# apache/skywalking-banyandb

Measured on NVIDIA H100. Metric: measure datapoints scanned+aggregated/sec, higher is better.
Workload: dtype f64

## Files before the change

### skywalking-banyandb_b200/csrc/capi.cu

```cuda
#include <cuda_runtime.h>
#include <unistd.h>

#include <algorithm>
#include <atomic>
#include <cstdio>
#include <chrono>
#include <condition_variable>
#include <cstddef>
#include <cstdlib>
#include <deque>
#include <functional>
#include <thread>
#include <future>
#include <cstring>
#include <memory>
#include <type_traits>
#include <mutex>
#include <optional>
#include <string>
#include <unordered_map>
#include <vector>

#include "../../include/bydb_gpu.h"
#include "part_dir.hpp"
// ... 48 lines not shown
    uint8_t *d_unpack = nullptr;
    uint64_t unpacked_pages = 0, unpack_skipped = 0;
    uint8_t *d_dense = nullptr;
    uint64_t dense_pages = 0, dense_bytes = 0;
    const DevBlock *d_blocks = nullptr;
    const DevCol *d_cols = nullptr;
    const uint8_t *const *d_files = nullptr;
    uint64_t hbm_bytes = 0;
    int device = 0;
    cudaStream_t pool_stream = nullptr;
    ~Part() {
        if (pool_stream) {
            if (d_arena) cudaFreeAsync(d_arena, pool_stream);
            if (d_dir) cudaFreeAsync(d_dir, pool_stream);
            if (d_unpack) cudaFreeAsync(d_unpack, pool_stream);
            if (d_dense) cudaFreeAsync(d_dense, pool_stream);
        } else {
            if (d_arena) cudaFree(d_arena);
            if (d_dir) cudaFree(d_dir);
            if (d_unpack) cudaFree(d_unpack);
            if (d_dense) cudaFree(d_dense);
        }
    }
};

struct ZeroPage {
    uint32_t work_count, work_next;
    uint32_t err[2];
    unsigned long long stats[6];
    int32_t col_type[kMaxFcols];
    unsigned long long dd_counts[2];
    uint32_t slow_count, slow_next;
    uint32_t rest_count, rest_next;
};
static_assert(offsetof(ZeroPage, err) == 8 && offsetof(ZeroPage, stats) == 16 && offsetof(ZeroPage, col_type) == 64 &&
                  offsetof(ZeroPage, dd_counts) == 96 && offsetof(ZeroPage, slow_count) == 112 && offsetof(ZeroPage, rest_count) == 120,
              "zero page layout");
constexpr size_t kZeroPageBytes = 256;
static_assert(sizeof(ZeroPage) <= kZeroPageBytes, "zero page size");

struct ExecSlot {
    cudaStream_t stream = nullptr;
    static constexpr int kMaxBatches = 8;
    cudaEvent_t ev[4 * kMaxBatches] = {};
    uint8_t *pinned = nullptr;
    size_t pinned_bytes = 0;
    uint8_t *zpage = nullptr;
    ZeroPage *page(int batch) { return reinterpret_cast<ZeroPage *>(zpage + kZeroPageBytes * static_cast<size_t>(batch)); }
    bool express[kMaxBatches] = {};
    cudaEvent_t busy = nullptr;
    bool busy_pending = false;
    void wait_idle() {
        if (busy_pending) cudaEventSynchronize(busy);
        busy_pending = false;
    }
    static constexpr size_t kInitialPinned = 1u << 20;
    std::vector<uint8_t *> retired;
    int ensure_pinned(size_t n) {
        if (n <= pinned_bytes) return 0;
        size_t want = align_up(std::max(n, 2 * pinned_bytes), 1 << 16);
        uint8_t *fresh = nullptr;
        if (cudaMallocHost(reinterpret_cast<void **>(&fresh), want) != cudaSuccess) {
            cudaGetLastError();
            want = align_up(n, 1 << 16);
            if (cudaMallocHost(reinterpret_cast<void **>(&fresh), want) != cudaSuccess) return -1;
        }
        if (pinned) retired.push_back(pinned);
        pinned = fresh;
        pinned_bytes = want;
// ... 78 lines not shown
constexpr int kCommMaxRanks = 64;
constexpr size_t kCommCtl = 4096, kCommStatusOff = 1024, kCommDoneOff = 2048, kCommErrOff = 2056, kCommArgsOff = 2112;
struct Comm {
    int rank = -1, nranks = 0;
    uint8_t *mine = nullptr;
    size_t slot_bytes = 0, mailbox_bytes = 0;
    std::vector<uint8_t *> peer;
    std::vector<bool> ipc_opened;
    std::vector<size_t> peer_slot_bytes;
    uint64_t epoch = 0;
    std::vector<uint64_t> last_use;
    std::mutex mu;
    bool shared_device = false;
    cudaStream_t poll_stream = nullptr;
    unsigned long long *poll_buf = nullptr;
};

struct StageRing {
    static constexpr int kBufs = 3;
    static constexpr size_t kBytes = 64u << 20;
    uint8_t *buf[kBufs] = {};
    cudaEvent_t done[kBufs] = {};
    bool pending[kBufs] = {};
    int next = 0;
    std::mutex mu;
};

struct bydb_ctx {
    int device = 0;
    int sm_count = 0;
    int ctas_per_sm = 2;
    int ctas_per_sm_fast = 2;
    int ctas_per_sm_express = 2;
    uint64_t hbm_budget = 0;
    uint64_t hbm_used = 0;
    bool host_index = false;
    bool dense_pages = true;
    std::mutex mu;
    NameTable names;
    std::unordered_map<bydb_part_h, std::shared_ptr<Part>> parts;
    std::unordered_map<uint64_t, bydb_part_h> by_id;
    std::atomic<uint64_t> parts_gen{0};
    bydb_part_h next_handle = 1;
    std::vector<std::unique_ptr<ExecSlot>> free_slots;
    WorkPool pool;
    Comm comm;
    StageRing stage;
};

namespace {

int hbm_reserve(bydb_ctx *ctx, uint64_t bytes, const char *msg = "HBM budget exceeded") {
    std::lock_guard<std::mutex> lk(ctx->mu);
    if (ctx->hbm_budget && ctx->hbm_used + bytes > ctx->hbm_budget) return fail(BYDB_ENOMEM, msg);
    ctx->hbm_used += bytes;
    return 0;
}
void hbm_release(bydb_ctx *ctx, uint64_t bytes) {
    std::lock_guard<std::mutex> lk(ctx->mu);
    ctx->hbm_used -= bytes;
}

struct SlotLease {
    bydb_ctx *ctx;
    std::unique_ptr<ExecSlot> slot;
    SlotLease(bydb_ctx *c) : ctx(c) {
// ... 851 lines not shown
        sp.dd_index = reinterpret_cast<int32_t *>(d + off_dd_index);
        sp.dd_row_off = reinterpret_cast<unsigned long long *>(d + off_dd_rowoff);
        sp.dd_list = reinterpret_cast<uint32_t *>(d + off_dd_list);
        sp.dd_counts = z->dd_counts;
        CUDA_TRY(cudaMemsetAsync(sp.dd_index, 0xff, NB * 4, stream));
        launch_detect_overlap(sp, stream);
        CUDA_TRY(cudaMemcpyAsync(hz->dd_counts, z->dd_counts, sizeof hz->dd_counts, cudaMemcpyDeviceToHost, stream));
        CUDA_TRY(cudaStreamSynchronize(stream));
        const unsigned long long n_ddb = hz->dd_counts[0], n_ddr = hz->dd_counts[1];
        extra_launches += 1;
        if (stats) stats->d2h_bytes += sizeof hz->dd_counts;
        if (n_ddb > 0) {
            const size_t b_ts = align_up(n_ddr * 8, 256), b_sh = align_up(n_ddb * kMaskWords * 4, 256);
            CUDA_TRY(dd_scratch.alloc(2 * b_ts + b_sh, stream));
            sp.dd_ts = reinterpret_cast<int64_t *>(dd_scratch.base);
            sp.dd_ver = reinterpret_cast<int64_t *>(dd_scratch.base + b_ts);
            sp.dd_shadow = reinterpret_cast<uint32_t *>(dd_scratch.base + 2 * b_ts);
            sp.n_dd_blocks = static_cast<uint32_t>(n_ddb);
            launch_dedup(sp, ctx->sm_count * ctx->ctas_per_sm, stream);
            extra_launches += 2;
        }
        rp.dedup_done = 1;
    }
    {
        bool sums_only = q->n_preds == 0 && !overlap && NB > 0;
        for (size_t c = 0; c < F; ++c) sums_only = sums_only && (sp.fcol_need[c] & 2) == 0;
        slot.express[batch] = sums_only;
        if (sums_only) {
            sp.rest_list = reinterpret_cast<uint32_t *>(d + off_restlist);
            sp.rest_count = &z->rest_count;
            sp.rest_next = &z->rest_next;
            if (stats) stats->kernel_launches += 1;
        }
    }
    CUDA_TRY(cudaEventRecord(ev[1], stream));
    launch_scan_blocks(sp, ctx->sm_count * ctx->ctas_per_sm_express, ctx->sm_count * ctx->ctas_per_sm_fast, ctx->sm_count * ctx->ctas_per_sm, stream);
    CUDA_TRY(cudaEventRecord(ev[2], stream));
    launch_series_reduce(rp, stream);
    const int32_t *gstart = reinterpret_cast<const int32_t *>(h + st.off_gstart);
    bool small_groups = true;
    for (int32_t g = 0; g < G && small_groups; ++g) small_groups = gstart[g + 1] - gstart[g] <= 32;
    launch_group_reduce(rp, stream, small_groups);
    CUDA_TRY(cudaEventRecord(ev[3], stream));
    if (!resident) CUDA_TRY(cudaMemcpyAsync(hz, z, kZeroPageBytes, cudaMemcpyDeviceToHost, stream));
    if (stats) {
        stats->kernel_launches += (NB ? 1u : 0u) + 2u + (NS ? 1u : 0u) + 1u + extra_launches;
        if (!resident) stats->d2h_bytes += kZeroPageBytes;
    }
    return 0;
}

int read_zero_page(const ZeroPage &z, bool express, bydb_stats *stats) {
    if (stats) {
        stats->rows_scanned += z.stats[0];
        stats->rows_matched += z.stats[1];
        stats->page_bytes += z.stats[2];
        stats->blocks_scanned += z.stats[3];
        stats->blocks_slow_lane += static_cast<uint32_t>(z.stats[4]);
        stats->slow_lane_reasons |= static_cast<uint32_t>(z.stats[5]);
        stats->blocks_express_lane += express ? z.work_count - z.rest_count : 0u;
    }
    if (z.err[0] == 0) return 0;
    g_last_dev_err = z.err[0];
    char buf[96];
    snprintf(buf, sizeof buf, " (block/series #%u)", z.err[1]);
    return fail(dev_err_code(z.err[0]), std::string(dev_err_text(z.err[0])) + buf);
}

int collect_scan(ExecSlot &slot, bydb_stats *stats, int batch = 0) {
// ... 1642 lines not shown
    if (prop.major != 9 || prop.minor != 0)
        return fail(BYDB_ENOTSUP, std::string("device '") + prop.name + "' is not sm_90 (Hopper); this library is built for sm_90a only");
    auto ctx = new bydb_ctx();
    ctx->device = dev;
    ctx->sm_count = prop.multiProcessorCount;
    ctx->hbm_budget = cfg ? cfg->hbm_budget_bytes : 0;
    ctx->host_index = cfg && (cfg->flags & BYDB_CFG_HOST_INDEX) != 0;
    ctx->dense_pages = !(cfg && (cfg->flags & BYDB_CFG_NO_DENSE_PAGES) != 0);
    if (upload_pow10_table()) {
        delete ctx;
        return fail(BYDB_EIO, "cannot upload constant tables (is the library built for this GPU?)");
    }
    {
        cudaMemPool_t pool;
        if (cudaDeviceGetDefaultMemPool(&pool, dev) == cudaSuccess) {
            uint64_t thr = UINT64_MAX;
            cudaMemPoolSetAttribute(pool, cudaMemPoolAttrReleaseThreshold, &thr);
            int no = 0;
            cudaMemPoolSetAttribute(pool, cudaMemPoolReuseAllowInternalDependencies, &no);
        }
    }
    for (int i = 0; i < 2; ++i) {
        std::unique_ptr<ExecSlot> sl(new ExecSlot());
        if (sl->create() != 0) {
            cudaGetLastError();
            break;
        }
        ctx->free_slots.push_back(std::move(sl));
    }
    preload_kernels();
    preload_unpack_kernels();
    preload_index_kernels();
    preload_encode_kernels();
    int occ_express = 1, occ_fast = 1, occ_slow = 1;
    scan_max_ctas_per_sm(&occ_express, &occ_fast, &occ_slow);
    int want = (cfg && cfg->warps_per_sm > 0) ? (cfg->warps_per_sm + kWarpsPerCta - 1) / kWarpsPerCta : 64;
    ctx->ctas_per_sm = std::max(1, std::min(want, occ_slow));
    ctx->ctas_per_sm_fast = std::max(1, std::min(want, occ_fast));
    ctx->ctas_per_sm_express = std::max(1, std::min(want, occ_express));
    *out = ctx;
    return 0;
    });
}

void bydb_shutdown(bydb_ctx *ctx) {
    if (!ctx) return;
    cudaSetDevice(ctx->device);
    cudaDeviceSynchronize();
    ctx->free_slots.clear();
    ctx->parts.clear();
    for (int i = 0; i < StageRing::kBufs; ++i) {
        if (ctx->stage.buf[i]) cudaFreeHost(ctx->stage.buf[i]);
        if (ctx->stage.done[i]) cudaEventDestroy(ctx->stage.done[i]);
    }
    for (size_t r = 0; r < ctx->comm.peer.size(); ++r)
        if (ctx->comm.ipc_opened[r] && ctx->comm.peer[r]) cudaIpcCloseMemHandle(ctx->comm.peer[r]);
    if (ctx->comm.mine) cudaFree(ctx->comm.mine);
    if (ctx->comm.poll_stream) cudaStreamDestroy(ctx->comm.poll_stream);
    if (ctx->comm.poll_buf) cudaFreeHost(ctx->comm.poll_buf);
    delete ctx;
}

int bydb_part_register(bydb_ctx *ctx, uint64_t part_id, const bydb_part_files *files, bydb_part_h *out) {
    return guarded([&]() -> int {
    if (!ctx || !out) return fail(BYDB_EINVAL, "ctx/out is NULL");
    {
        std::lock_guard<std::mutex> lk(ctx->mu);
        auto it = ctx->by_id.find(part_id);
        if (it != ctx->by_id.end()) {
            *out = it->second;
            return 0;
        }
// ... 1718 lines not shown
```

### skywalking-banyandb_b200/csrc/scan_kernels.cu

```cuda
#include "scan_kernels.cuh"
#include "lane_decode.cuh"

#include <atomic>
#include <cfloat>
#include <cmath>
#include <cstring>

#include "../../include/bydb_gpu.h"

namespace bydb {

__constant__ double c_pow10[309];

__device__ __forceinline__ uint32_t smem_u32(const void *p) { return static_cast<uint32_t>(__cvta_generic_to_shared(p)); }

__device__ __forceinline__ void mbar_init(uint64_t *bar, uint32_t count) {
    asm volatile("mbarrier.init.shared::cta.b64 [%0], %1;" ::"r"(smem_u32(bar)), "r"(count) : "memory");
}
__device__ __forceinline__ void mbar_expect_tx(uint64_t *bar, uint32_t bytes) {
    asm volatile("mbarrier.arrive.expect_tx.shared::cta.b64 _, [%0], %1;" ::"r"(smem_u32(bar)), "r"(bytes) : "memory");
}
__device__ __forceinline__ bool mbar_try_wait(uint64_t *bar, uint32_t parity) {
    uint32_t ok;
    asm volatile(
// ... 1963 lines not shown
    swar_begin(sl, pw);
#pragma unroll
    for (int q = 0; q < 2; ++q) {
        const uint4 wa = *reinterpret_cast<const uint4 *>(src + 32 * q), wb = *reinterpret_cast<const uint4 *>(src + 32 * q + 16);
        swar_step<kClasses, false>(sl, wa.x, 0u);
        swar_step<kClasses, false>(sl, wa.y, 0u);
        swar_step<kClasses, false>(sl, wa.z, 0u);
        swar_step<kClasses, false>(sl, wa.w, 0u);
        swar_step<kClasses, false>(sl, wb.x, 0u);
        swar_step<kClasses, false>(sl, wb.y, 0u);
        swar_step<kClasses, false>(sl, wb.z, 0u);
        swar_step<kClasses, false>(sl, wb.w, 0u);
    }
}
struct ExpressUnit {
    int32_t Ta, Ra, Tb, Rb;
    uint32_t n;
    bool wide;
};
template <int kClasses>
__device__ __forceinline__ ExpressUnit express_unit(const uint8_t *src, uint32_t pwa, uint32_t pwb) {
    ExpressUnit r;
    SwarLane sl;
    express_half<kClasses>(sl, src, pwa);
    uint32_t wide = sl.wide;
    const uint32_t na = swar_end(sl, r.Ta, r.Ra);
    express_half<kClasses>(sl, src + kSwarChunkBytes, pwb);
    wide |= sl.wide;
    r.n = na | (swar_end(sl, r.Tb, r.Rb) << 16);
    r.wide = __any_sync(0xffffffffu, (wide & 0x80808080u) != 0);
    return r;
}

__global__ void __launch_bounds__(kWarpsPerCta * 32, BYDB_EXPRESS_CTAS) scan_sum_express_kernel(const __grid_constant__ ScanParams p) {
    extern __shared__ __align__(128) uint8_t smem_raw[];
    const int lane = threadIdx.x & 31;
    const int warp = threadIdx.x >> 5;
    ExpressSmem *sm = reinterpret_cast<ExpressSmem *>(smem_raw) + warp;
    if (lane == 0) {
        sm->fault = 0;
        for (int s = 0; s < kExpressStages; ++s) mbar_init(&sm->bar[s], 1);
        asm volatile("fence.mbarrier_init.release.cluster;" ::: "memory");
    }
    __syncthreads();
    const uint32_t nwork = *p.work_count;
    uint32_t seq = 0;
    unsigned long long st_rows = 0, st_bytes = 0;
    uint32_t st_blocks = 0, known_types = 0;
    for (;;) {
        uint32_t nb = 0;
        const uint32_t base = grab_work(p.work_next, nwork, kExpressBatch, nb, lane);
        if (nb == 0) break;
        const bool mine = static_cast<uint32_t>(lane) < nb;
        uint32_t g = 0, count = 0, col_begin = 0, n_cols = 0, pi = 0;
        bool ok = mine;
        if (mine) {
            g = p.worklist[base + lane];
            while (pi + 1 < p.n_parts && g >= p.parts[pi + 1].block_base) ++pi;
            const DevBlock *b = p.parts[pi].blocks + (g - p.parts[pi].block_base);
            count = b->count;
            col_begin = b->col_begin;
            n_cols = b->n_cols;
            ok = p.tmin <= b->ts_min && p.tmax >= b->ts_max && count >= 1;
        }
        uint32_t page_bytes = 0;
        for (uint32_t c = 0; c < p.n_fcols; ++c) {
            const uint8_t *abase = nullptr;
            uint32_t pstart = 0, pend = 0, total = 0, nst = 0, dense_b = 0;
            int64_t first = 0;
            int exp = 0;
            bool has_page = false, is_float = false, count_only = false, dense = false;
            if (ok) {
                const DevCol *cols = p.parts[pi].cols + col_begin;
                DevCol col{};
                bool found = false;
                uint32_t ci = 0;
                for (uint32_t i = 0; i < n_cols && !found; ++i) {
                    const DevCol cc = cols[i];
                    if (cc.name_id == p.fcol_name[c]) {
                        col = cc;
                        found = true;
                        ci = i;
                    }
                }
                if (found) {
                    is_float = col.value_type == BYDB_VT_FLOAT64;
                    if (!is_float && col.value_type != BYDB_VT_INT64) {
                        ok = false;
                    } else if (!check_col_type(p, c, col.value_type, known_types)) {
                        ok = false;
                    }
                    const uint8_t *page = p.parts[pi].files[col.file_id] + col.off;
                    const uint32_t hdr = is_float ? 11u : 9u;
                    if (ok && p.fcol_need[c] == 0) {
                        if (col.size < 2 || __ldg(page) == 9 || (__ldg(page) == kEncRawCells && __ldg(page + 1))) ok = false;
                        count_only = ok;
                        page_bytes += 1;
                    } else if (ok && p.parts[pi].dense && p.parts[pi].dense[col_begin + ci].n == count) {
                        const DevDense dd = p.parts[pi].dense[col_begin + ci];
                        exp = dd.exp;
                        first = dd.min;
                        dense_b = dd.b;
                        abase = dd.planes;
                        pend = total = dd.plane_bytes;
                        nst = (total + kExpressStageBytes - 1) / kExpressStageBytes;
                        has_page = true;
                        dense = true;
                        page_bytes += col.size;
                    } else if (ok) {
                        if (col.size < hdr || __ldg(page) != 3) {
                            ok = false;
                        } else {
                            if (is_float) exp = static_cast<int16_t>((static_cast<uint32_t>(__ldg(page + 1)) << 8) | __ldg(page + 2));
                            first = conv_bytes_to_int64(page + hdr - 8);
                            const uintptr_t a = reinterpret_cast<uintptr_t>(page + hdr);
                            abase = reinterpret_cast<const uint8_t *>(a & ~static_cast<uintptr_t>(15));
                            pstart = static_cast<uint32_t>(a & 15);
                            pend = pstart + (col.size - hdr);
                            total = (pend + 15u) & ~15u;
                            nst = pend > pstart ? (total + kExpressStageBytes - 1) / kExpressStageBytes : 0;
                            has_page = true;
                            page_bytes += col.size;
                        }
                    }
                }
            }
            const bool streams = ok && has_page && nst > 0;
            uint32_t sb = streams ? nst : 0;
#pragma unroll
            for (int sft = 1; sft < static_cast<int>(kExpressBatch); sft <<= 1) {
                const uint32_t o = __shfl_up_sync(0xffffffffu, sb, sft);
                if (lane >= sft) sb += o;
            }
            const uint32_t ts = __shfl_sync(0xffffffffu, sb, kExpressBatch - 1);
            sb -= streams ? nst : 0;
            const uint32_t seq0 = seq;
            auto issue = [&](uint32_t s) {
                const uint32_t bal = __ballot_sync(0xffffffffu, streams && s >= sb && s < sb + nst);
                const int src = __ffs(bal) - 1;
                const uint64_t ab = shfl_u64(reinterpret_cast<uint64_t>(abase), src);
                const uint32_t tot = __shfl_sync(0xffffffffu, total, src);
                const uint32_t off = (s - __shfl_sync(0xffffffffu, sb, src)) * kExpressStageBytes;
                if (lane == 0) ring_fill(sm, seq0 + s, reinterpret_cast<const uint8_t *>(ab) + off, min(static_cast<uint32_t>(kExpressStageBytes), tot - off));
            };
            __syncwarp();
            for (uint32_t s = 0; s < ts && s < static_cast<uint32_t>(kExpressStages); ++s) issue(s);
            seq += ts;
            for (uint32_t k = 0; k < nb; ++k) {
                const bool okk = __shfl_sync(0xffffffffu, ok, k);
                if (!okk) continue;
                const bool pagek = __shfl_sync(0xffffffffu, has_page, k);
                const bool cok = __shfl_sync(0xffffffffu, count_only, k);
                const uint32_t count_k = __shfl_sync(0xffffffffu, count, k);
                AggAcc acc;
                acc.init();
                bool good = true;
                if (pagek) {
                    const uint32_t nst_k = __shfl_sync(0xffffffffu, nst, k), sb_k = __shfl_sync(0xffffffffu, sb, k);
                    const uint32_t ps_k = __shfl_sync(0xffffffffu, pstart, k), pe_k = __shfl_sync(0xffffffffu, pend, k);
// ... 54 lines not shown
#endif
                        }
                        if (!dense_k && j == nst_k - 1 && lane == 0) last_byte = buf[(pe_k - 1) % kExpressStageBytes];
                        __syncwarp();
                        const uint32_t nx = s + kExpressStages;
                        if (nx < ts) {
                            if (j + kExpressStages < nst_k) {
                                const uint32_t off = (j + kExpressStages) * kExpressStageBytes;
                                if (lane == 0) ring_fill(sm, seq0 + nx, ab_k + off, min(static_cast<uint32_t>(kExpressStageBytes), tot_k - off));
                            } else {
                                issue(nx);
                            }
                        }
                    }
                    last_byte = __shfl_sync(0xffffffffu, last_byte, 0);
                    const int32_t zeros_after = static_cast<int32_t>(nst_k * kExpressStageBytes - pe_k);
                    if (dense_k) good = true;
                    else if (nst_k == 0) good = count_k == 1;
                    else good = good && tb - zeros_after + 1 == static_cast<int32_t>(count_k) && last_byte < 0x80u;
#if !BYDB_EXPRESS_DECODE
                    good = true;
#endif
                    uint64_t us = U + static_cast<uint64_t>(S);
#pragma unroll
                    for (int m = 16; m >= 1; m >>= 1) us += shfl_xor_u64(us, m);
                    acc.add_scaled(first_k, count_k);
                    acc.lo += us;
                    acc.hi += (dense_k ? 0 : (static_cast<int64_t>(us) >> 63)) + (acc.lo < us ? 1 : 0);
                    acc.cnt = count_k;
                } else if (cok) {
                    acc.cnt = count_k;
                }
                if (static_cast<uint32_t>(lane) == k) {
                    if (!good) {
                        ok = false;
                    } else {
                        BlockPartial bp;
                        bp.sum.i = 0;
                        bp.mn.i = 0;
                        bp.mx.i = 0;
                        bp.cnt = acc.cnt;
                        if (acc.cnt > 0 && is_float) {
                            double sd;
                            if (acc.hi == (static_cast<int64_t>(acc.lo) >> 63)) sd = __ll2double_rn(static_cast<int64_t>(acc.lo));
                            else sd = __ll2double_rn(acc.hi) * 18446744073709551616.0 + __ull2double_rn(acc.lo);
                            bp.sum.f = scale_decimal(sd, exp);
                            bp.mn.f = scale_decimal(__ll2double_rn(acc.mn), exp);
                            bp.mx.f = scale_decimal(__ll2double_rn(acc.mx), exp);
                        } else if (acc.cnt > 0) {
                            bp.sum.i = static_cast<int64_t>(acc.lo);
                            bp.mn.i = acc.mn;
                            bp.mx.i = acc.mx;
                        }
                        p.P[static_cast<size_t>(g) * p.n_fcols + c] = bp;
                    }
                }
            }
        }
        const bool done = mine && ok;
        if (done) p.Prows[g] = count;
        const uint32_t rows_sum = __reduce_add_sync(0xffffffffu, done ? count : 0u);
        const uint32_t bytes_sum = __reduce_add_sync(0xffffffffu, done ? page_bytes : 0u);
        const uint32_t done_bal = __ballot_sync(0xffffffffu, done), rest_bal = __ballot_sync(0xffffffffu, mine && !ok);
        uint32_t rbase = 0;
        st_rows += rows_sum;
        st_bytes += bytes_sum;
        st_blocks += __popc(done_bal);
        if (lane == 0 && rest_bal) rbase = atomicAdd(p.rest_count, static_cast<uint32_t>(__popc(rest_bal)));
        rbase = __shfl_sync(0xffffffffu, rbase, 0);
        if (mine && !ok) p.rest_list[rbase + __popc(rest_bal & ((1u << lane) - 1u))] = g;
    }
    if (lane == 0 && st_blocks) {
        atomicAdd(&p.stats[0], st_rows);
        atomicAdd(&p.stats[1], st_rows);
        atomicAdd(&p.stats[2], st_bytes);
        atomicAdd(&p.stats[3], static_cast<unsigned long long>(st_blocks));
    }
    if (sm->fault && lane == 0) atomicCAS(&p.err[0], 0u, static_cast<uint32_t>(kErrTmaTimeout));
}


__device__ __forceinline__ WarpSmem *dense_warp_init(int lane) {
    extern __shared__ __align__(128) uint8_t smem_raw[];
    WarpSmem *sm = reinterpret_cast<WarpSmem *>(smem_raw) + (threadIdx.x >> 5);
    if (lane == 0) {
        sm->fault = 0;
        sm->seq = 0;
        for (int s = 0; s < kStages; ++s) mbar_init(&sm->bar[s], 1);
        asm volatile("fence.mbarrier_init.release.cluster;" ::: "memory");
    }
    __syncthreads();
    return sm;
}
__device__ __forceinline__ uint32_t dense_page_hdr(const DenseParams &p, const DevCol &col, const uint8_t *&page) {
    if (col.file_id != p.fv_file_id || (col.value_type != BYDB_VT_INT64 && col.value_type != BYDB_VT_FLOAT64)) return 0;
    const uint32_t hdr = col.value_type == BYDB_VT_FLOAT64 ? 11u : 9u;
    page = p.files[col.file_id] + col.off;
    return col.size >= hdr && __ldg(page) == 3 ? hdr : 0;
}

__global__ void __launch_bounds__(kWarpsPerCta * 32) dense_classify_kernel(const __grid_constant__ DenseParams p) {
    const int lane = threadIdx.x & 31;
    WarpSmem *sm = dense_warp_init(lane);
    for (uint32_t bi = blockIdx.x * kWarpsPerCta + (threadIdx.x >> 5); bi < p.n_blocks; bi += gridDim.x * kWarpsPerCta) {
        const DevBlock blk = p.blocks[bi];
        if (blk.count == 0 || blk.count > kDenseMaxRows) continue;
        for (uint32_t c = 0; c < blk.n_cols; ++c) {
            const uint32_t ci = blk.col_begin + c;
            const DevCol col = p.cols[ci];
            const uint8_t *page = nullptr;
            const uint32_t hdr = dense_page_hdr(p, col, page);
// ... 2865 lines not shown
    n += 2;
    for (uint32_t size = 4096; size <= N; size <<= 1) {
        for (uint32_t j = size >> 1; j >= 2048; j >>= 1, ++n) bitonic_step_kernel<<<N / 2 / 256, 256, 0, s>>>(p.keys, j, size, N / 2);
        bitonic_tile_kernel<<<N / 2048, 1024, 0, s>>>(p.keys, size, size);
        n += 1;
    }
    wide_comp_place_kernel<<<(n_comp + 255) / 256, 256, 0, s>>>(p, n_comp);
    launch_excl_scan(p.seg, nr, p.tiles, &p.ctl[0] + 4, s);
    wide_comp_order_kernel<<<(p.n_rows + 255) / 256, 256, 0, s>>>(p);
    const uint64_t words = (7ull * p.F + 1) * n_comp + p.F;
    wide_comp_fold_kernel<<<static_cast<unsigned>((words + 255) / 256), 256, 0, s>>>(p, n_comp);
    return n + 6;
}

void launch_plan_blocks(const ScanParams &p, cudaStream_t s) {
    if (p.total_blocks == 0) return;
    const int threads = 256;
    plan_blocks_kernel<<<(p.total_blocks + threads - 1) / threads, threads, 0, s>>>(p);
}

static std::atomic<bool> g_attr_set[64];
static void scan_set_attrs() {
    int dev = 0;
    cudaGetDevice(&dev);
    if (dev >= 0 && dev < 64 && g_attr_set[dev].load(std::memory_order_acquire)) return;
    const int smem = static_cast<int>(scan_smem_bytes());
    cudaFuncSetAttribute(scan_blocks_kernel<true>, cudaFuncAttributeMaxDynamicSharedMemorySize, smem);
    cudaFuncSetAttribute(scan_blocks_kernel<false>, cudaFuncAttributeMaxDynamicSharedMemorySize, smem);
    cudaFuncSetAttribute(scan_sum_express_kernel, cudaFuncAttributeMaxDynamicSharedMemorySize, static_cast<int>(express_smem_bytes()));
    cudaFuncSetAttribute(dedup_kernel, cudaFuncAttributeMaxDynamicSharedMemorySize, smem);
    cudaFuncSetAttribute(key_values_i64_kernel, cudaFuncAttributeMaxDynamicSharedMemorySize, smem + static_cast<int>(kKeyCacheBytes));
    if (dev >= 0 && dev < 64) g_attr_set[dev].store(true, std::memory_order_release);
}
void launch_scan_blocks(const ScanParams &p, int grid_express, int grid_fast, int grid_slow, cudaStream_t s) {
    scan_set_attrs();
    const size_t smem = scan_smem_bytes();
    if (p.rest_list) scan_sum_express_kernel<<<grid_express, kWarpsPerCta * 32, express_smem_bytes(), s>>>(p);
    scan_blocks_kernel<true><<<grid_fast, kWarpsPerCta * 32, smem, s>>>(p);
    scan_blocks_kernel<false><<<grid_slow, kWarpsPerCta * 32, smem, s>>>(p);
}

void launch_dense_classify(const DenseParams &p, int grid, cudaStream_t s) {
    cudaFuncSetAttribute(dense_classify_kernel, cudaFuncAttributeMaxDynamicSharedMemorySize, static_cast<int>(scan_smem_bytes()));
    dense_classify_kernel<<<grid, kWarpsPerCta * 32, scan_smem_bytes(), s>>>(p);
}
void launch_dense_write(const DenseParams &p, int grid, cudaStream_t s) {
    cudaFuncSetAttribute(dense_write_kernel, cudaFuncAttributeMaxDynamicSharedMemorySize, static_cast<int>(scan_smem_bytes()));
    dense_write_kernel<<<grid, kWarpsPerCta * 32, scan_smem_bytes(), s>>>(p);
}

void scan_max_ctas_per_sm(int *express, int *fast, int *slow) {
    scan_set_attrs();
    int e = 1, a = 1, b = 1;
    cudaOccupancyMaxActiveBlocksPerMultiprocessor(&e, scan_sum_express_kernel, kWarpsPerCta * 32, express_smem_bytes());
    cudaOccupancyMaxActiveBlocksPerMultiprocessor(&a, scan_blocks_kernel<true>, kWarpsPerCta * 32, scan_smem_bytes());
    cudaOccupancyMaxActiveBlocksPerMultiprocessor(&b, scan_blocks_kernel<false>, kWarpsPerCta * 32, scan_smem_bytes());
    *express = e < 1 ? 1 : e;
    *fast = a < 1 ? 1 : a;
    *slow = b < 1 ? 1 : b;
}

void launch_detect_overlap(const ScanParams &p, cudaStream_t s) {
    if (p.n_series == 0) return;
    const int threads = 128;
    detect_overlap_kernel<<<(p.n_series + threads - 1) / threads, threads, 0, s>>>(p);
}
void launch_dedup(const ScanParams &p, int grid, cudaStream_t s) {
    if (p.n_dd_blocks == 0) return;
    const size_t smem = scan_smem_bytes();
    scan_set_attrs();
    dedup_kernel<<<grid, kWarpsPerCta * 32, smem, s>>>(p, 0);
    dedup_kernel<<<grid, kWarpsPerCta * 32, smem, s>>>(p, 1);
}
void launch_series_reduce(const ReduceParams &p, cudaStream_t s) {
    if (p.n_series == 0) return;
    const int threads = 256;
    series_reduce_kernel<<<(p.n_series + 7) / 8, threads, 0, s>>>(p);
}
void launch_group_reduce(const ReduceParams &p, cudaStream_t s, bool small_groups) {
    if (p.n_groups <= 0) return;
    if (small_groups) group_reduce_small_kernel<<<(p.n_groups + 7) / 8, 256, 0, s>>>(p);
    else group_reduce_kernel<<<p.n_groups, 256, 0, s>>>(p);
}
void launch_combine_tables(uint8_t *tables, uint32_t n_tables, const TableLayout &tl, cudaStream_t s, size_t stride_bytes) {
    const uint64_t words = tl.total / 8;
    if (words == 0 || n_tables < 2) return;
// ... 91 lines not shown
    launch_select_rows(p, s);
    return 2;
}
void launch_finalize(const FinalizeParams &p, cudaStream_t s) {
    const int threads = 128;
    const int n = p.n_groups > 0 ? p.n_groups : 1;
    finalize_kernel<<<(n + threads - 1) / threads, threads, 0, s>>>(p);
}

void preload_kernels() {
    cudaFuncAttributes ka;
    (void)cudaFuncGetAttributes(&ka, key_values_kernel);
    (void)cudaFuncGetAttributes(&ka, key_pack_kernel);
    (void)cudaFuncGetAttributes(&ka, key_values_i64_kernel);
    (void)cudaFuncGetAttributes(&ka, key_pack_i64_kernel);
    (void)cudaFuncGetAttributes(&ka, key_order_kernel);
    (void)cudaFuncGetAttributes(&ka, key_perm_kernel);
    (void)cudaFuncGetAttributes(&ka, permute_table_kernel);
    (void)cudaFuncGetAttributes(&ka, keyed_partial_rows_kernel);
    (void)cudaFuncGetAttributes(&ka, present_groups_kernel);
    (void)cudaFuncGetAttributes(&ka, rows_to_host_kernel);
    (void)cudaFuncGetAttributes(&ka, key_union_kernel);
    (void)cudaFuncGetAttributes(&ka, rank_span_check_kernel);
    (void)cudaFuncGetAttributes(&ka, combine_keyed_kernel);
    (void)cudaFuncGetAttributes(&ka, merge_first_kernel);
    cudaFuncAttributes a;
    cudaFuncGetAttributes(&a, step_reset_kernel);
    cudaFuncGetAttributes(&a, keyed_step_reset_kernel);
    cudaFuncGetAttributes(&a, keyed_row_map_kernel);
    cudaFuncGetAttributes(&a, plan_blocks_kernel);
    cudaFuncGetAttributes(&a, scan_blocks_kernel<true>);
    cudaFuncGetAttributes(&a, scan_blocks_kernel<false>);
    cudaFuncGetAttributes(&a, scan_sum_express_kernel);
    cudaFuncGetAttributes(&a, dense_classify_kernel);
    cudaFuncGetAttributes(&a, dense_write_kernel);
    cudaFuncGetAttributes(&a, detect_overlap_kernel);
    cudaFuncGetAttributes(&a, dedup_kernel);
    cudaFuncGetAttributes(&a, series_reduce_kernel);
    cudaFuncGetAttributes(&a, group_reduce_kernel);
    cudaFuncGetAttributes(&a, group_reduce_small_kernel);
    cudaFuncGetAttributes(&a, finalize_kernel);
    cudaFuncGetAttributes(&a, select_rows_kernel<true>);
    cudaFuncGetAttributes(&a, select_rows_kernel<false>);
    cudaFuncGetAttributes(&a, combine_tables_kernel);
    cudaFuncGetAttributes(&a, comm_wait_kernel);
    cudaFuncGetAttributes(&a, comm_signal_kernel);
    cudaFuncGetAttributes(&a, comm_wait_args_kernel);
    cudaFuncGetAttributes(&a, comm_signal_args_kernel);
    cudaFuncGetAttributes(&a, comm_done_args_kernel);
    cudaGetLastError();
}

int upload_pow10_table() {
    static const double tab[32] = {1e00, 1e01, 1e02, 1e03, 1e04, 1e05, 1e06, 1e07, 1e08, 1e09, 1e10,
                                   1e11, 1e12, 1e13, 1e14, 1e15, 1e16, 1e17, 1e18, 1e19, 1e20, 1e21,
                                   1e22, 1e23, 1e24, 1e25, 1e26, 1e27, 1e28, 1e29, 1e30, 1e31};
    static const double postab32[10] = {1e00, 1e32, 1e64, 1e96, 1e128, 1e160, 1e192, 1e224, 1e256, 1e288};
    double h[309];
    for (int n = 0; n <= 308; ++n) {
        volatile double a = postab32[n / 32], b = tab[n % 32];
        volatile double r = a * b;
        h[n] = r;
    }
    return cudaMemcpyToSymbol(c_pow10, h, sizeof(h)) == cudaSuccess ? 0 : -1;
}

// ... 2 lines not shown
```

### skywalking-banyandb_b200/csrc/scan_kernels.cuh

```cuda
#pragma once

#include <cuda_runtime.h>

#include <cstdint>

#include "../../include/bydb_gpu.h"
#include "dense_page.cuh"
#include "part_dir.hpp"

namespace bydb {

constexpr int kWarpsPerCta = 8;
#ifndef BYDB_STAGE_BYTES
#define BYDB_STAGE_BYTES 2048
#endif
#ifndef BYDB_STAGES
#define BYDB_STAGES 2
#endif
#ifndef BYDB_EXPRESS_STAGES
#define BYDB_EXPRESS_STAGES 2
#endif
#ifndef BYDB_EXPRESS_CTAS
#define BYDB_EXPRESS_CTAS 2
#endif
#ifndef BYDB_EXPRESS_DECODE
#define BYDB_EXPRESS_DECODE 1
#endif
#ifndef BYDB_FAST_CTAS
#define BYDB_FAST_CTAS 3
#endif
constexpr int kStageBytes = BYDB_STAGE_BYTES;
constexpr int kStages = BYDB_STAGES;
constexpr int kChunkBytes = 512;
constexpr int kMaskWords = 264;
constexpr int kMaxFcols = 8;
constexpr int kMaxPreds = 8;
constexpr int kMaxLit = 64;
constexpr int kMaxParts = 64;

enum DevErr : uint32_t {
    kErrNone = 0,
    kErrPlainPage = 1,
    kErrZstdDict = 2,
    kErrBigBlock = 3,
    kErrCorrupt = 4,
    kErrTypeMix = 5,
    kErrBadEnc = 6,
    kErrTagPlain = 7,
    kErrOverlap = 8,
    kErrPredType = 9,
    kErrTmaTimeout = 10,
    kErrPeerTimeout = 11,
    kErrKeyCap = 12,
    kErrKeyLong = 13,
    kErrRankOverlap = 14,
    kErrKeyBlock = 15,
    kErrTupleBlock = 16,
};
constexpr int kOpEqOrNil = 7;
// ... 16 lines not shown
    uint8_t value_type;
    uint8_t lit[kMaxLit];
};

struct BlockPartial {
    union { double f; int64_t i; } sum, mn, mx;
    int64_t cnt;
};
static_assert(sizeof(BlockPartial) == 32, "BlockPartial layout");

__host__ __device__ __forceinline__ bool met_column(bool is_float, int64_t cnt, int64_t max_i64, double max_f64) {
    return cnt > 0 || (is_float ? max_i64 == 0 : max_f64 == 0.0);
}

struct ScanParams {
    DevPartRef parts[kMaxParts];
    uint32_t n_parts;
    uint32_t total_blocks;
    const uint64_t *q_sids;
    uint32_t n_series;
    uint32_t n_fcols;
    uint32_t n_preds;
    uint32_t pad0;
    int64_t tmin, tmax;
    uint16_t fcol_name[kMaxFcols];
    uint8_t fcol_need[kMaxFcols];
    DevPred preds[kMaxPreds];
    uint32_t *worklist;
    uint32_t *work_count;
    uint32_t *work_next;
    uint32_t *rest_list;
    uint32_t *rest_count;
    uint32_t *rest_next;
    uint32_t *slow_list;
    uint32_t *slow_count;
    uint32_t *slow_next;
    int32_t *block_qsid;
    uint32_t *first_block;
    BlockPartial *P;
    uint32_t *Prows;
    uint32_t *Pfirst;
    int32_t *col_type;
    uint32_t *err;
    unsigned long long *stats;
    int32_t *dd_index;
    unsigned long long *dd_row_off;
    uint32_t *dd_list;
    unsigned long long *dd_counts;
    int64_t *dd_ts, *dd_ver;
    uint32_t *dd_shadow;
    uint32_t n_dd_blocks;
    uint32_t pad1;
};

static_assert(sizeof(ScanParams) + 256 <= 4096, "ScanParams (with WideScanParams beside it) must fit the 4 KB kernel-parameter space");

struct ReduceParams {
    DevPartRef parts[kMaxParts];
    uint32_t n_parts;
    uint32_t n_series;
    uint32_t n_fcols;
    int32_t n_groups;
    const uint64_t *q_sids;
    const int32_t *order;
    const int32_t *group_start;
    const int32_t *block_qsid;
// ... 387 lines not shown
    const uint8_t *const *files;
    DevDense *dense;
    uint32_t n_blocks;
    uint32_t fv_file_id;
    unsigned long long *counters;
    uint8_t *arena;
    uint32_t *scratch;
    uint32_t scratch_rows;
    uint32_t pad;
};
void launch_dense_classify(const DenseParams &p, int grid, cudaStream_t s);
void launch_dense_write(const DenseParams &p, int grid, cudaStream_t s);

struct EncodeParams {
    const void *values;
    const uint64_t *block_off;
    uint32_t n_blocks;
    uint32_t is_float;
    int64_t *scratch;
    int16_t *exps;
    uint8_t *slots;
    const uint64_t *slot_off;
    uint32_t *page_len;
    uint8_t *status;
};
void launch_encode_pages(const EncodeParams &p, int grid, cudaStream_t s);
void launch_gather_pages(const EncodeParams &p, const uint64_t *out_off, uint8_t *out, int grid, cudaStream_t s);
void preload_encode_kernels();

size_t scan_smem_bytes();
size_t express_smem_bytes();
void launch_plan_blocks(const ScanParams &p, cudaStream_t s);
void launch_step_reset(uint32_t *zero_page, uint32_t *first_block, size_t n_first, cudaStream_t s);
void launch_scan_blocks(const ScanParams &p, int grid_express, int grid_fast, int grid_slow, cudaStream_t s);
void launch_series_reduce(const ReduceParams &p, cudaStream_t s);
void launch_group_reduce(const ReduceParams &p, cudaStream_t s, bool small_groups = false);
void launch_finalize(const FinalizeParams &p, cudaStream_t s);
void launch_detect_overlap(const ScanParams &p, cudaStream_t s);
void launch_dedup(const ScanParams &p, int grid, cudaStream_t s);
int upload_pow10_table();
void scan_max_ctas_per_sm(int *express, int *fast, int *slow);
void preload_kernels();
void preload_unpack_kernels();
void preload_index_kernels();

}
```

Before: 1540 billion.

## Add dense-page streaming sum kernel ahead of express lane with overflow ring

Adds a TMA-free dense sum kernel for sums-only queries over dense-paged parts. Warps stream bit-plane data with double-buffered non-caching vector loads and prefetch the next work batch. Blocks it cannot handle are pushed to a ring list, which the express kernel then consumes instead of the main worklist. This avoids the express kernel's mbarrier/TMA staging overhead for dense pages, at the cost of an extra launch and reusing the slow-list buffer as ring storage.

```diff
diff --git a/skywalking-banyandb_b200/csrc/capi.cu b/skywalking-banyandb_b200/csrc/capi.cu
--- a/skywalking-banyandb_b200/csrc/capi.cu
+++ b/skywalking-banyandb_b200/csrc/capi.cu
@@ -104,9 +104,11 @@
     unsigned long long dd_counts[2];
     uint32_t slow_count, slow_next;
     uint32_t rest_count, rest_next;
+    uint32_t ring_count, ring_next;
 };
 static_assert(offsetof(ZeroPage, err) == 8 && offsetof(ZeroPage, stats) == 16 && offsetof(ZeroPage, col_type) == 64 &&
-                  offsetof(ZeroPage, dd_counts) == 96 && offsetof(ZeroPage, slow_count) == 112 && offsetof(ZeroPage, rest_count) == 120,
+                  offsetof(ZeroPage, dd_counts) == 96 && offsetof(ZeroPage, slow_count) == 112 && offsetof(ZeroPage, rest_count) == 120 &&
+                  offsetof(ZeroPage, ring_count) == 128,
               "zero page layout");
 constexpr size_t kZeroPageBytes = 256;
 static_assert(sizeof(ZeroPage) <= kZeroPageBytes, "zero page size");
@@ -251,6 +253,7 @@
     int ctas_per_sm = 2;
     int ctas_per_sm_fast = 2;
     int ctas_per_sm_express = 2;
+    int ctas_per_sm_dense = 2;
     uint64_t hbm_budget = 0;
     uint64_t hbm_used = 0;
     bool host_index = false;
@@ -1168,9 +1171,17 @@
             sp.rest_next = &z->rest_next;
             if (stats) stats->kernel_launches += 1;
         }
+        bool dense = false;
+        for (uint32_t i = 0; i < sp.n_parts; ++i) dense = dense || sp.parts[i].dense != nullptr;
+        if (dense && sums_only && ctx->ctas_per_sm_dense > 0) {
+            sp.ring_list = reinterpret_cast<uint32_t *>(d + off_slowlist);
+            sp.ring_count = &z->ring_count;
+            sp.ring_next = &z->ring_next;
+            if (stats) stats->kernel_launches += 1;
+        }
     }
     CUDA_TRY(cudaEventRecord(ev[1], stream));
-    launch_scan_blocks(sp, ctx->sm_count * ctx->ctas_per_sm_express, ctx->sm_count * ctx->ctas_per_sm_fast, ctx->sm_count * ctx->ctas_per_sm, stream);
+    launch_scan_blocks(sp, ctx->sm_count * ctx->ctas_per_sm_dense, ctx->sm_count * ctx->ctas_per_sm_express, ctx->sm_count * ctx->ctas_per_sm_fast, ctx->sm_count * ctx->ctas_per_sm, stream);
     CUDA_TRY(cudaEventRecord(ev[2], stream));
     launch_series_reduce(rp, stream);
     const int32_t *gstart = reinterpret_cast<const int32_t *>(h + st.off_gstart);
@@ -2879,12 +2890,13 @@
     preload_unpack_kernels();
     preload_index_kernels();
     preload_encode_kernels();
-    int occ_express = 1, occ_fast = 1, occ_slow = 1;
-    scan_max_ctas_per_sm(&occ_express, &occ_fast, &occ_slow);
+    int occ_dense = 1, occ_express = 1, occ_fast = 1, occ_slow = 1;
+    scan_max_ctas_per_sm(&occ_dense, &occ_express, &occ_fast, &occ_slow);
     int want = (cfg && cfg->warps_per_sm > 0) ? (cfg->warps_per_sm + kWarpsPerCta - 1) / kWarpsPerCta : 64;
     ctx->ctas_per_sm = std::max(1, std::min(want, occ_slow));
     ctx->ctas_per_sm_fast = std::max(1, std::min(want, occ_fast));
     ctx->ctas_per_sm_express = std::max(1, std::min(want, occ_express));
+    ctx->ctas_per_sm_dense = occ_dense > 0 ? std::max(1, std::min(want, occ_dense)) : 0;
     *out = ctx;
     return 0;
     });
diff --git a/skywalking-banyandb_b200/csrc/scan_kernels.cu b/skywalking-banyandb_b200/csrc/scan_kernels.cu
--- a/skywalking-banyandb_b200/csrc/scan_kernels.cu
+++ b/skywalking-banyandb_b200/csrc/scan_kernels.cu
@@ -2019,99 +2019,139 @@
     return r;
 }
 
+__device__ __forceinline__ bool express_block(const ScanParams &p, uint32_t g, uint32_t &pi, uint32_t &count, uint32_t &col_begin, uint32_t &n_cols) {
+    pi = 0;
+    while (pi + 1 < p.n_parts && g >= p.parts[pi + 1].block_base) ++pi;
+    const DevBlock *b = p.parts[pi].blocks + (g - p.parts[pi].block_base);
+    count = b->count;
+    col_begin = b->col_begin;
+    n_cols = b->n_cols;
+    return p.tmin <= b->ts_min && p.tmax >= b->ts_max && count >= 1;
+}
+struct ExpressPage {
+    const uint8_t *abase = nullptr;
+    uint32_t pstart = 0, pend = 0, total = 0, nst = 0, dense_b = 0;
+    int64_t first = 0;
+    int exp = 0;
+    bool has_page = false, is_float = false, count_only = false, dense = false;
+};
+__device__ __forceinline__ ExpressPage express_page(const ScanParams &p, uint32_t pi, uint32_t col_begin, uint32_t n_cols, uint32_t count, uint32_t c,
+                                                    uint32_t &known_types, bool &ok, uint32_t &page_bytes) {
+    ExpressPage e;
+    const DevCol *cols = p.parts[pi].cols + col_begin;
+    DevCol col{};
+    bool found = false;
+    uint32_t ci = 0;
+    for (uint32_t i = 0; i < n_cols && !found; ++i) {
+        const DevCol cc = cols[i];
+        if (cc.name_id == p.fcol_name[c]) {
+            col = cc;
+            found = true;
+            ci = i;
+        }
+    }
+    if (!found) return e;
+    e.is_float = col.value_type == BYDB_VT_FLOAT64;
+    if (!e.is_float && col.value_type != BYDB_VT_INT64) {
+        ok = false;
+    } else if (!check_col_type(p, c, col.value_type, known_types)) {
+        ok = false;
+    }
+    const uint8_t *page = p.parts[pi].files[col.file_id] + col.off;
+    const uint32_t hdr = e.is_float ? 11u : 9u;
+    if (ok && p.fcol_need[c] == 0) {
+        if (col.size < 2 || __ldg(page) == 9 || (__ldg(page) == kEncRawCells && __ldg(page + 1))) ok = false;
+        e.count_only = ok;
+        page_bytes += 1;
+    } else if (ok && p.parts[pi].dense && p.parts[pi].dense[col_begin + ci].n == count) {
+        const DevDense dd = p.parts[pi].dense[col_begin + ci];
+        e.exp = dd.exp;
+        e.first = dd.min;
+        e.dense_b = dd.b;
+        e.abase = dd.planes;
+        e.pend = e.total = dd.plane_bytes;
+        e.nst = (e.total + kExpressStageBytes - 1) / kExpressStageBytes;
+        e.has_page = true;
+        e.dense = true;
+        page_bytes += col.size;
+    } else if (ok) {
+        if (col.size < hdr || __ldg(page) != 3) {
+            ok = false;
+        } else {
+            if (e.is_float) e.exp = static_cast<int16_t>((static_cast<uint32_t>(__ldg(page + 1)) << 8) | __ldg(page + 2));
+            e.first = conv_bytes_to_int64(page + hdr - 8);
+            const uintptr_t a = reinterpret_cast<uintptr_t>(page + hdr);
+            e.abase = reinterpret_cast<const uint8_t *>(a & ~static_cast<uintptr_t>(15));
+            e.pstart = static_cast<uint32_t>(a & 15);
+            e.pend = e.pstart + (col.size - hdr);
+            e.total = (e.pend + 15u) & ~15u;
+            e.nst = e.pend > e.pstart ? (e.total + kExpressStageBytes - 1) / kExpressStageBytes : 0;
+            e.has_page = true;
+            page_bytes += col.size;
+        }
+    }
+    return e;
+}
+__device__ __forceinline__ BlockPartial express_partial(const AggAcc &acc, bool is_float, int exp) {
+    BlockPartial bp;
+    bp.sum.i = 0;
+    bp.mn.i = 0;
+    bp.mx.i = 0;
+    bp.cnt = acc.cnt;
+    if (acc.cnt > 0 && is_float) {
+        double sd;
+        if (acc.hi == (static_cast<int64_t>(acc.lo) >> 63)) sd = __ll2double_rn(static_cast<int64_t>(acc.lo));
+        else sd = __ll2double_rn(acc.hi) * 18446744073709551616.0 + __ull2double_rn(acc.lo);
+        bp.sum.f = scale_decimal(sd, exp);
+        bp.mn.f = scale_decimal(__ll2double_rn(acc.mn), exp);
+        bp.mx.f = scale_decimal(__ll2double_rn(acc.mx), exp);
+    } else if (acc.cnt > 0) {
+        bp.sum.i = static_cast<int64_t>(acc.lo);
+        bp.mn.i = acc.mn;
+        bp.mx.i = acc.mx;
+    }
+    return bp;
+}
+
 __global__ void __launch_bounds__(kWarpsPerCta * 32, BYDB_EXPRESS_CTAS) scan_sum_express_kernel(const __grid_constant__ ScanParams p) {
     extern __shared__ __align__(128) uint8_t smem_raw[];
     const int lane = threadIdx.x & 31;
     const int warp = threadIdx.x >> 5;
     ExpressSmem *sm = reinterpret_cast<ExpressSmem *>(smem_raw) + warp;
+    const bool after_dense = p.ring_list != nullptr;
+    const uint32_t nwork = after_dense ? *p.ring_count : *p.work_count;
+    if (nwork == 0) return;
     if (lane == 0) {
         sm->fault = 0;
         for (int s = 0; s < kExpressStages; ++s) mbar_init(&sm->bar[s], 1);
         asm volatile("fence.mbarrier_init.release.cluster;" ::: "memory");
     }
     __syncthreads();
-    const uint32_t nwork = *p.work_count;
+    const uint32_t *list = after_dense ? p.ring_list : p.worklist;
+    uint32_t *cursor = after_dense ? p.ring_next : p.work_next;
     uint32_t seq = 0;
     unsigned long long st_rows = 0, st_bytes = 0;
     uint32_t st_blocks = 0, known_types = 0;
     for (;;) {
         uint32_t nb = 0;
-        const uint32_t base = grab_work(p.work_next, nwork, kExpressBatch, nb, lane);
+        const uint32_t base = grab_work(cursor, nwork, kExpressBatch, nb, lane);
         if (nb == 0) break;
         const bool mine = static_cast<uint32_t>(lane) < nb;
         uint32_t g = 0, count = 0, col_begin = 0, n_cols = 0, pi = 0;
         bool ok = mine;
         if (mine) {
-            g = p.worklist[base + lane];
-            while (pi + 1 < p.n_parts && g >= p.parts[pi + 1].block_base) ++pi;
-            const DevBlock *b = p.parts[pi].blocks + (g - p.parts[pi].block_base);
-            count = b->count;
-            col_begin = b->col_begin;
-            n_cols = b->n_cols;
-            ok = p.tmin <= b->ts_min && p.tmax >= b->ts_max && count >= 1;
+            g = list[base + lane];
+            ok = express_block(p, g, pi, count, col_begin, n_cols);
         }
         uint32_t page_bytes = 0;
         for (uint32_t c = 0; c < p.n_fcols; ++c) {
-            const uint8_t *abase = nullptr;
-            uint32_t pstart = 0, pend = 0, total = 0, nst = 0, dense_b = 0;
-            int64_t first = 0;
-            int exp = 0;
-            bool has_page = false, is_float = false, count_only = false, dense = false;
-            if (ok) {
-                const DevCol *cols = p.parts[pi].cols + col_begin;
-                DevCol col{};
-                bool found = false;
-                uint32_t ci = 0;
-                for (uint32_t i = 0; i < n_cols && !found; ++i) {
-                    const DevCol cc = cols[i];
-                    if (cc.name_id == p.fcol_name[c]) {
-                        col = cc;
-                        found = true;
-                        ci = i;
-                    }
-                }
-                if (found) {
-                    is_float = col.value_type == BYDB_VT_FLOAT64;
-                    if (!is_float && col.value_type != BYDB_VT_INT64) {
-                        ok = false;
-                    } else if (!check_col_type(p, c, col.value_type, known_types)) {
-                        ok = false;
-                    }
-                    const uint8_t *page = p.parts[pi].files[col.file_id] + col.off;
-                    const uint32_t hdr = is_float ? 11u : 9u;
-                    if (ok && p.fcol_need[c] == 0) {
-                        if (col.size < 2 || __ldg(page) == 9 || (__ldg(page) == kEncRawCells && __ldg(page + 1))) ok = false;
-                        count_only = ok;
-                        page_bytes += 1;
-                    } else if (ok && p.parts[pi].dense && p.parts[pi].dense[col_begin + ci].n == count) {
-                        const DevDense dd = p.parts[pi].dense[col_begin + ci];
-                        exp = dd.exp;
-                        first = dd.min;
-                        dense_b = dd.b;
-                        abase = dd.planes;
-                        pend = total = dd.plane_bytes;
-                        nst = (total + kExpressStageBytes - 1) / kExpressStageBytes;
-                        has_page = true;
-                        dense = true;
-                        page_bytes += col.size;
-                    } else if (ok) {
-                        if (col.size < hdr || __ldg(page) != 3) {
-                            ok = false;
-                        } else {
-                            if (is_float) exp = static_cast<int16_t>((static_cast<uint32_t>(__ldg(page + 1)) << 8) | __ldg(page + 2));
-                            first = conv_bytes_to_int64(page + hdr - 8);
-                            const uintptr_t a = reinterpret_cast<uintptr_t>(page + hdr);
-                            abase = reinterpret_cast<const uint8_t *>(a & ~static_cast<uintptr_t>(15));
-                            pstart = static_cast<uint32_t>(a & 15);
-                            pend = pstart + (col.size - hdr);
-                            total = (pend + 15u) & ~15u;
-                            nst = pend > pstart ? (total + kExpressStageBytes - 1) / kExpressStageBytes : 0;
-                            has_page = true;
-                            page_bytes += col.size;
-                        }
-                    }
-                }
-            }
+            ExpressPage pg;
+            if (ok) pg = express_page(p, pi, col_begin, n_cols, count, c, known_types, ok, page_bytes);
+            const uint8_t *const abase = pg.abase;
+            const uint32_t pstart = pg.pstart, pend = pg.pend, total = pg.total, nst = pg.nst, dense_b = pg.dense_b;
+            const int64_t first = pg.first;
+            const int exp = pg.exp;
+            const bool has_page = pg.has_page, is_float = pg.is_float, count_only = pg.count_only, dense = pg.dense;
             const bool streams = ok && has_page && nst > 0;
             uint32_t sb = streams ? nst : 0;
 #pragma unroll
@@ -2232,28 +2272,8 @@
                     acc.cnt = count_k;
                 }
                 if (static_cast<uint32_t>(lane) == k) {
-                    if (!good) {
-                        ok = false;
-                    } else {
-                        BlockPartial bp;
-                        bp.sum.i = 0;
-                        bp.mn.i = 0;
-                        bp.mx.i = 0;
-                        bp.cnt = acc.cnt;
-                        if (acc.cnt > 0 && is_float) {
-                            double sd;
-                            if (acc.hi == (static_cast<int64_t>(acc.lo) >> 63)) sd = __ll2double_rn(static_cast<int64_t>(acc.lo));
-                            else sd = __ll2double_rn(acc.hi) * 18446744073709551616.0 + __ull2double_rn(acc.lo);
-                            bp.sum.f = scale_decimal(sd, exp);
-                            bp.mn.f = scale_decimal(__ll2double_rn(acc.mn), exp);
-                            bp.mx.f = scale_decimal(__ll2double_rn(acc.mx), exp);
-                        } else if (acc.cnt > 0) {
-                            bp.sum.i = static_cast<int64_t>(acc.lo);
-                            bp.mn.i = acc.mn;
-                            bp.mx.i = acc.mx;
-                        }
-                        p.P[static_cast<size_t>(g) * p.n_fcols + c] = bp;
-                    }
+                    if (!good) ok = false;
+                    else p.P[static_cast<size_t>(g) * p.n_fcols + c] = express_partial(acc, is_float, exp);
                 }
             }
         }
@@ -2277,6 +2297,142 @@
         atomicAdd(&p.stats[3], static_cast<unsigned long long>(st_blocks));
     }
     if (sm->fault && lane == 0) atomicCAS(&p.err[0], 0u, static_cast<uint32_t>(kErrTmaTimeout));
+}
+
+constexpr int kDenseCtaThreads = 256;
+constexpr int kDenseMinCtas = BYDB_DENSE_CTAS;
+constexpr uint32_t kDenseGrab = 32;
+constexpr int kDenseLoads = BYDB_DENSE_LOADS;
+constexpr uint32_t kDenseChunkBytes = 32u * kDenseLoads * 16u;
+
+__device__ __forceinline__ uint4 ld_stream_v4(const uint8_t *a) {
+    uint4 v;
+    asm("ld.global.nc.L1::no_allocate.v4.u32 {%0, %1, %2, %3}, [%4];" : "=r"(v.x), "=r"(v.y), "=r"(v.z), "=r"(v.w) : "l"(a));
+    return v;
+}
+__device__ __forceinline__ void dense_load_chunk(uint4 (&v)[kDenseLoads], const uint8_t *src, uint32_t off, uint32_t tot, int lane) {
+#pragma unroll
+    for (int q = 0; q < kDenseLoads; ++q) {
+        const uint32_t o = off + 16u * (static_cast<uint32_t>(lane) + 32u * q);
+        v[q] = o < tot ? ld_stream_v4(src + o) : make_uint4(0u, 0u, 0u, 0u);
+    }
+}
+
+__global__ void __launch_bounds__(kDenseCtaThreads, kDenseMinCtas) scan_sum_dense_kernel(const __grid_constant__ ScanParams p) {
+    const int lane = threadIdx.x & 31;
+    const uint32_t nwork = *p.work_count;
+    unsigned long long st_rows = 0, st_bytes = 0;
+    uint32_t st_blocks = 0, known_types = 0;
+    uint32_t nb = 0;
+    const uint32_t base0 = grab_work(p.work_next, nwork, kDenseGrab, nb, lane);
+    uint32_t g_next = static_cast<uint32_t>(lane) < nb ? p.worklist[base0 + lane] : 0u;
+    for (;;) {
+        if (nb == 0) break;
+        uint32_t nb2 = 0, g_next2 = 0;
+        bool grabbed = false;
+        auto grab_next = [&]() {
+            const uint32_t base2 = grab_work(p.work_next, nwork, kDenseGrab, nb2, lane);
+            g_next2 = static_cast<uint32_t>(lane) < nb2 ? p.worklist[base2 + lane] : 0u;
+            grabbed = true;
+        };
+        const bool mine = static_cast<uint32_t>(lane) < nb;
+        uint32_t g = 0, count = 0, col_begin = 0, n_cols = 0, pi = 0, page_bytes = 0;
+        bool ok = mine;
+        if (mine) {
+            g = g_next;
+            ok = express_block(p, g, pi, count, col_begin, n_cols);
+        }
+        for (uint32_t c = 0; c < p.n_fcols && ok; ++c) {
+            const ExpressPage pg = express_page(p, pi, col_begin, n_cols, count, c, known_types, ok, page_bytes);
+            ok = ok && (pg.dense || pg.count_only);
+        }
+        for (uint32_t c = 0; c < p.n_fcols; ++c) {
+            ExpressPage pg;
+            if (ok) {
+                bool again = true;
+                uint32_t counted = 0;
+                pg = express_page(p, pi, col_begin, n_cols, count, c, known_types, again, counted);
+            }
+            const bool streams = ok && pg.dense && pg.total > 0;
+            uint64_t own = 0;
+            uint32_t todo = __ballot_sync(0xffffffffu, streams);
+            if (todo) {
+                int k = __ffs(todo) - 1;
+                const uint8_t *src = reinterpret_cast<const uint8_t *>(shfl_u64(reinterpret_cast<uint64_t>(pg.abase), k));
+                uint32_t tot = __shfl_sync(0xffffffffu, pg.total, k), b = __shfl_sync(0xffffffffu, pg.dense_b, k), off = 0;
+                uint32_t end[kDensePlanes];
+                dense_plane_ends(__shfl_sync(0xffffffffu, count, k), b, end);
+                uint4 v[kDenseLoads];
+                dense_load_chunk(v, src, 0, tot, lane);
+                if (!grabbed) grab_next();
+                uint64_t U = 0;
+                for (;;) {
+                    uint32_t noff = off + kDenseChunkBytes, ntot = tot;
+                    int nk = k;
+                    const uint8_t *nsrc = src;
+                    if (noff >= tot) {
+                        todo &= todo - 1u;
+                        nk = todo ? __ffs(todo) - 1 : -1;
+                        noff = 0;
+                        ntot = 0;
+                        if (nk >= 0) {
+                            nsrc = reinterpret_cast<const uint8_t *>(shfl_u64(reinterpret_cast<uint64_t>(pg.abase), nk));
+                            ntot = __shfl_sync(0xffffffffu, pg.total, nk);
+                        }
+                    }
+                    uint4 w[kDenseLoads];
+                    dense_load_chunk(w, nsrc, noff, ntot, lane);
+#pragma unroll
+                    for (int q = 0; q < kDenseLoads; ++q) U += dense_piece_sum(v[q], off + 16u * (static_cast<uint32_t>(lane) + 32u * q), end, b);
+                    if (nk != k) {
+#pragma unroll
+                        for (int m = 16; m >= 1; m >>= 1) U += shfl_xor_u64(U, m);
+                        if (lane == k) own = U;
+                        if (nk < 0) break;
+                        U = 0;
+                        b = __shfl_sync(0xffffffffu, pg.dense_b, nk);
+                        dense_plane_ends(__shfl_sync(0xffffffffu, count, nk), b, end);
+                    }
+#pragma unroll
+                    for (int q = 0; q < kDenseLoads; ++q) v[q] = w[q];
+                    off = noff;
+                    k = nk;
+                    src = nsrc;
+                    tot = ntot;
+                }
+            }
+            if (ok) {
+                AggAcc acc;
+                acc.init();
+                if (pg.dense) {
+                    acc.add_scaled(pg.first, count);
+                    acc.lo += own;
+                    acc.hi += acc.lo < own ? 1 : 0;
+                }
+                acc.cnt = count;
+                p.P[static_cast<size_t>(g) * p.n_fcols + c] = express_partial(acc, pg.is_float, pg.exp);
+            }
+        }
+        const bool done = mine && ok;
+        if (done) p.Prows[g] = count;
+        st_rows += __reduce_add_sync(0xffffffffu, done ? count : 0u);
+        st_bytes += __reduce_add_sync(0xffffffffu, done ? page_bytes : 0u);
+        const uint32_t done_bal = __ballot_sync(0xffffffffu, done), left_bal = __ballot_sync(0xffffffffu, mine && !ok);
+        st_blocks += __popc(done_bal);
+        uint32_t rbase = 0;
+        if (lane == 0 && left_bal) rbase = atomicAdd(p.ring_count, static_cast<uint32_t>(__popc(left_bal)));
+        rbase = __shfl_sync(0xffffffffu, rbase, 0);
+        if (mine && !ok) p.ring_list[rbase + __popc(left_bal & ((1u << lane) - 1u))] = g;
+        if (!grabbed) grab_next();
+        nb = nb2;
+        g_next = g_next2;
+    }
+    if (lane == 0 && st_blocks) {
+        atomicAdd(&p.stats[0], st_rows);
+        atomicAdd(&p.stats[1], st_rows);
+        atomicAdd(&p.stats[2], st_bytes);
+        atomicAdd(&p.stats[3], static_cast<unsigned long long>(st_blocks));
+    }
 }
 
 
@@ -5208,9 +5364,10 @@
     cudaFuncSetAttribute(key_values_i64_kernel, cudaFuncAttributeMaxDynamicSharedMemorySize, smem + static_cast<int>(kKeyCacheBytes));
     if (dev >= 0 && dev < 64) g_attr_set[dev].store(true, std::memory_order_release);
 }
-void launch_scan_blocks(const ScanParams &p, int grid_express, int grid_fast, int grid_slow, cudaStream_t s) {
+void launch_scan_blocks(const ScanParams &p, int grid_dense, int grid_express, int grid_fast, int grid_slow, cudaStream_t s) {
     scan_set_attrs();
     const size_t smem = scan_smem_bytes();
+    if (p.ring_list) scan_sum_dense_kernel<<<grid_dense, kDenseCtaThreads, 0, s>>>(p);
     if (p.rest_list) scan_sum_express_kernel<<<grid_express, kWarpsPerCta * 32, express_smem_bytes(), s>>>(p);
     scan_blocks_kernel<true><<<grid_fast, kWarpsPerCta * 32, smem, s>>>(p);
     scan_blocks_kernel<false><<<grid_slow, kWarpsPerCta * 32, smem, s>>>(p);
@@ -5225,9 +5382,11 @@
     dense_write_kernel<<<grid, kWarpsPerCta * 32, scan_smem_bytes(), s>>>(p);
 }
 
-void scan_max_ctas_per_sm(int *express, int *fast, int *slow) {
+void scan_max_ctas_per_sm(int *dense, int *express, int *fast, int *slow) {
     scan_set_attrs();
-    int e = 1, a = 1, b = 1;
+    int d = 1, e = 1, a = 1, b = 1;
+    cudaOccupancyMaxActiveBlocksPerMultiprocessor(&d, scan_sum_dense_kernel, kDenseCtaThreads, 0);
+    *dense = BYDB_DENSE_LANE ? (d < 1 ? 1 : d) : 0;
     cudaOccupancyMaxActiveBlocksPerMultiprocessor(&e, scan_sum_express_kernel, kWarpsPerCta * 32, express_smem_bytes());
     cudaOccupancyMaxActiveBlocksPerMultiprocessor(&a, scan_blocks_kernel<true>, kWarpsPerCta * 32, scan_smem_bytes());
     cudaOccupancyMaxActiveBlocksPerMultiprocessor(&b, scan_blocks_kernel<false>, kWarpsPerCta * 32, scan_smem_bytes());
@@ -5385,6 +5544,7 @@
     cudaFuncGetAttributes(&a, scan_blocks_kernel<true>);
     cudaFuncGetAttributes(&a, scan_blocks_kernel<false>);
     cudaFuncGetAttributes(&a, scan_sum_express_kernel);
+    cudaFuncGetAttributes(&a, scan_sum_dense_kernel);
     cudaFuncGetAttributes(&a, dense_classify_kernel);
     cudaFuncGetAttributes(&a, dense_write_kernel);
     cudaFuncGetAttributes(&a, detect_overlap_kernel);
diff --git a/skywalking-banyandb_b200/csrc/scan_kernels.cuh b/skywalking-banyandb_b200/csrc/scan_kernels.cuh
--- a/skywalking-banyandb_b200/csrc/scan_kernels.cuh
+++ b/skywalking-banyandb_b200/csrc/scan_kernels.cuh
@@ -25,6 +25,15 @@
 #endif
 #ifndef BYDB_EXPRESS_DECODE
 #define BYDB_EXPRESS_DECODE 1
+#endif
+#ifndef BYDB_DENSE_LANE
+#define BYDB_DENSE_LANE 1
+#endif
+#ifndef BYDB_DENSE_CTAS
+#define BYDB_DENSE_CTAS 2
+#endif
+#ifndef BYDB_DENSE_LOADS
+#define BYDB_DENSE_LOADS 8
 #endif
 #ifndef BYDB_FAST_CTAS
 #define BYDB_FAST_CTAS 3
@@ -107,6 +116,9 @@
     uint32_t *rest_list;
     uint32_t *rest_count;
     uint32_t *rest_next;
+    uint32_t *ring_list;
+    uint32_t *ring_count;
+    uint32_t *ring_next;
     uint32_t *slow_list;
     uint32_t *slow_count;
     uint32_t *slow_next;
@@ -560,14 +572,14 @@
 size_t express_smem_bytes();
 void launch_plan_blocks(const ScanParams &p, cudaStream_t s);
 void launch_step_reset(uint32_t *zero_page, uint32_t *first_block, size_t n_first, cudaStream_t s);
-void launch_scan_blocks(const ScanParams &p, int grid_express, int grid_fast, int grid_slow, cudaStream_t s);
+void launch_scan_blocks(const ScanParams &p, int grid_dense, int grid_express, int grid_fast, int grid_slow, cudaStream_t s);
 void launch_series_reduce(const ReduceParams &p, cudaStream_t s);
 void launch_group_reduce(const ReduceParams &p, cudaStream_t s, bool small_groups = false);
 void launch_finalize(const FinalizeParams &p, cudaStream_t s);
 void launch_detect_overlap(const ScanParams &p, cudaStream_t s);
 void launch_dedup(const ScanParams &p, int grid, cudaStream_t s);
 int upload_pow10_table();
-void scan_max_ctas_per_sm(int *express, int *fast, int *slow);
+void scan_max_ctas_per_sm(int *dense, int *express, int *fast, int *slow);
 void preload_kernels();
 void preload_unpack_kernels();
 void preload_index_kernels();
```

Result: no change. 1560 billion, median of 6 (+1.3%).
